# warwick-hpsc/MG-CFD-app-plain

Hardware: AMD Instinct MI355X
Metric: Medges/s (compute_flux_edge) + MG V-cycle wall-s (higher is better)
Workload: dtype f64; 1 GPU; M6-L0-like synthetic level (67^3 jittered lattice, permuted ids): 300763 nodes / 888822 internal edges per GPU, flux + update sweep, no MG; numerics=exact (bit-identical to the reference), parallelism=1 GPU, workload_kind=level0

## Files before the change

include/mgcfd.h:

```cpp
#ifndef MGCFD_H
#define MGCFD_H

#include <stdint.h>

#ifdef __cplusplus
extern "C" {
#endif

#define MGCFD_NVAR 5
#define MGCFD_RK 3

#define MGCFD_MESH_FVCORR 0
#define MGCFD_MESH_M6_WING 2
#define MGCFD_MESH_LA_CASCADE 3
#define MGCFD_MESH_ROTOR_37 4

#define MGCFD_OK 0
#define MGCFD_ERR_ARG 1
#define MGCFD_ERR_IO 2
#define MGCFD_ERR_HIP 3
#define MGCFD_ERR_NAN 4
#define MGCFD_ERR_NEG_DENSITY 5
#define MGCFD_ERR_NEG_ENERGY 6
#define MGCFD_ERR_VALIDATION 7
// ... 1 lines not shown
enum { MGCFD_LOOP_FLUX = 0, MGCFD_LOOP_UPDATE, MGCFD_LOOP_COMPUTE_STEP, MGCFD_LOOP_TIME_STEP,
       MGCFD_LOOP_RESTRICT, MGCFD_LOOP_PROLONG, MGCFD_LOOP_INDIRECT_RW, MGCFD_NUM_LOOPS };

enum { MGCFD_ARR_VARIABLES = 0, MGCFD_ARR_OLD_VARIABLES, MGCFD_ARR_FLUXES, MGCFD_ARR_RESIDUALS,
       MGCFD_ARR_STEP_FACTORS, MGCFD_ARR_VOLUMES,
       MGCFD_ARR_STAGE  };

enum {
    MGCFD_OPT_EXACT = 0,
    MGCFD_OPT_TIMING = 1,
    MGCFD_OPT_INDIRECT_RW = 2,
    MGCFD_OPT_CHECK_INVALID = 3,
    MGCFD_OPT_FLUX_VARIANT = 4,
    MGCFD_OPT_FUSE_UPDATE = 5,
    MGCFD_OPT_GRAPH = 6,
    MGCFD_OPT_RANK_SPLIT = 7
};

typedef struct { int64_t a, b; double x, y, z; } mgcfd_edge;

typedef struct {
    int64_t nel;
    int64_t n_edges;
    int64_t n_internal, n_boundary, n_wall;
    int64_t internal_start, boundary_start, wall_start;
    const double *volumes;
    const double *coords;
    const mgcfd_edge *edges;
    const int64_t *mg_map;
    int64_t mgc;
} mgcfd_level_desc;
// ... 20 lines not shown

int mgcfd_create(const mgcfd_level_desc *levels, int nlevels, int mesh_variant, int device,
                 mgcfd_solver **out);
int mgcfd_create_from_mesh(const mgcfd_mesh *m, int device, mgcfd_solver **out);
int mgcfd_create_partitioned(const mgcfd_level_desc *levels, int nlevels, int mesh_variant, int device,
                             const int64_t *n_owned, mgcfd_solver **out);
int mgcfd_create_partitioned_mg(const mgcfd_level_desc *levels, int nlevels, int mesh_variant, int device,
                                const int64_t *n_owned, const int64_t *const *order_keys, mgcfd_solver **out);
int mgcfd_plan_audit(const mgcfd_level_desc *levels, int nlevels, int mesh_variant, const int64_t *n_owned,
                     const int64_t *const *order_keys, char *report, int64_t report_cap);
void mgcfd_destroy(mgcfd_solver *s);
int mgcfd_set_option(mgcfd_solver *s, int option, int value);
int mgcfd_level_has_edge_once(const mgcfd_solver *s, int level, int *yes);
int mgcfd_level_has_half_rows(const mgcfd_solver *s, int level, int *yes);
int mgcfd_level_has_order_free(const mgcfd_solver *s, int level, int *yes);
int mgcfd_level_tiling(const mgcfd_solver *s, int level, int64_t out[10]);
int mgcfd_get_option(const mgcfd_solver *s, int option, int *value);
int mgcfd_set_stream(mgcfd_solver *s, void *hip_stream);
int mgcfd_synchronize(mgcfd_solver *s);
int mgcfd_num_levels(const mgcfd_solver *s);
int64_t mgcfd_level_nel(const mgcfd_solver *s, int level);
int64_t mgcfd_level_num_internal_edges(const mgcfd_solver *s, int level);
int mgcfd_get_far_field(const mgcfd_solver *s, double *out17);

int mgcfd_copy_old_variables(mgcfd_solver *s, int level);
int mgcfd_compute_step_factor(mgcfd_solver *s, int level);
int mgcfd_compute_flux_edge(mgcfd_solver *s, int level);
int mgcfd_compute_boundary_flux_edge(mgcfd_solver *s, int level);
int mgcfd_compute_wall_flux_edge(mgcfd_solver *s, int level);
int mgcfd_compute_fluxes(mgcfd_solver *s, int level);
// ... 78 lines not shown
```

mg-cfd-app-plain_amd/csrc/device_plan.hpp:

```cpp
#pragma once

#include <hip/hip_runtime.h>
#include <cstdint>

#include "preprocess.hpp"

namespace mgcfd {

constexpr int kNumStateFields = 5;
static_assert(sizeof(EdgeW) == 32, "EdgeW must be 32 bytes");
static_assert(sizeof(ProlongW) == 24, "ProlongW must be 24 bytes");

struct FarField {
    double var[5];
    double fc_mx[3], fc_my[3], fc_mz[3], fc_de[3];
};

constexpr int kMaxPushPeers = 8;
struct PushPeers {
    double *base[kMaxPushPeers] = {nullptr, nullptr, nullptr, nullptr, nullptr, nullptr, nullptr, nullptr};
    int64_t stride[kMaxPushPeers] = {0, 0, 0, 0, 0, 0, 0, 0};
    int64_t first[kMaxPushPeers + 1] = {0, 0, 0, 0, 0, 0, 0, 0, 0};
    int n = 0;
};

struct PushFlags {
// ... 96 lines not shown
    int64_t n_edges = 0, n_edges_pad = 0;
    int32_t *fe_ab = nullptr, *row_edge = nullptr;
    double *fe_w = nullptr, *edge_flux = nullptr;
    int32_t *old_of_new = nullptr;
    int32_t *child_ptr = nullptr, *child = nullptr;
    int32_t *child4 = nullptr;
    double *pro_w = nullptr;
    int32_t *pro_p = nullptr;
    int pro_tiled = 0;
    int32_t *pro_tile_n = nullptr, *pro_tile_ids = nullptr;
    uint16_t *pro_s16 = nullptr, *pro_own16 = nullptr;
    int32_t *pro_parent = nullptr;
    double *pro_wsum = nullptr;
};

}
```

mg-cfd-app-plain_amd/csrc/kernels.hip:

```cpp
#include <hip/hip_runtime.h>
#include <algorithm>
#include <cstdlib>
#include <stdexcept>
#include <stdint.h>

#include "device_plan.hpp"

#ifndef MGCFD_KERNEL_NS
#error "compile with -DMGCFD_KERNEL_NS=exact|fast"
#endif

namespace mgcfd {
namespace MGCFD_KERNEL_NS {

#ifdef MGCFD_PHASES
__device__ unsigned long long g_phase[4096 * 8];
__device__ unsigned long long g_phase_abs[4096 * 8];
#define PH_MARK(k) do { if (threadIdx.x == 0) { unsigned long long now_ = wall_clock64(); g_phase[(blockIdx.x & 4095) * 8 + (k)] += now_ - ph_last_; ph_last_ = now_; g_phase_abs[(blockIdx.x & 4095) * 8 + 1 + (k)] = now_; } } while (0)
#define PH_BEGIN() unsigned long long ph_last_ = wall_clock64(); if (threadIdx.x == 0) { g_phase[(blockIdx.x & 4095) * 8 + 7] += 1ull; g_phase_abs[(blockIdx.x & 4095) * 8] = ph_last_; \
        g_phase_abs[(blockIdx.x & 4095) * 8 + 7] = (static_cast<unsigned long long>(__builtin_amdgcn_s_getreg(20 | (0 << 6) | (31 << 11))) << 32) | __builtin_amdgcn_s_getreg(4 | (0 << 6) | (31 << 11)); }
#else
#define PH_MARK(k) do { } while (0)
#define PH_BEGIN() do { } while (0)
#endif
// ... 79 lines not shown
}

__device__ __forceinline__ NodeQ lds_load_record(const double2 *tile, uint32_t slot)
{
    const uint32_t b = (slot >> 3) & 1u;
    const double2 *even = tile + slot * kLdsRecD2 + b;
    const double2 *odd = tile + slot * kLdsRecD2 - b;
    const double2 a = even[0], bq = odd[1], c = even[2], d = odd[3], e = even[4];
    const double f = odd[5].x;
    NodeQ r;
    r.rho = a.x; r.mx = a.y; r.my = bq.x; r.mz = bq.y; r.en = c.x; r.vx = c.y;
    r.vy = d.x; r.vz = d.y; r.p = e.x; r.speed = e.y; r.c = f;
    return r;
}

struct FluxC { double xx, xy, xz, yy, yz, zz, ex, ey, ez; };

__device__ __forceinline__ FluxC flux_contribution(const NodeQ &q)
{
    FluxC f;
    f.xx = q.vx * q.mx + q.p;
    f.xy = q.vx * q.my;
    f.xz = q.vx * q.mz;
    f.yy = q.vy * q.my + q.p;
    f.yz = q.vy * q.mz;
    f.zz = q.vz * q.mz + q.p;
    const double de_p = q.en + q.p;
    f.ex = q.vx * de_p;
    f.ey = q.vy * de_p;
    f.ez = q.vz * de_p;
// ... 321 lines not shown
        } else if (e.code == kT16Far && (classes & 4)) {
            a0 += fx * (ff.var[1] + me.mx) + fy * (ff.var[2] + me.my) + fz * (ff.var[3] + me.mz);
            a4 += fx * (ff.fc_de[0] + fm.ex) + fy * (ff.fc_de[1] + fm.ey) + fz * (ff.fc_de[2] + fm.ez);
            a1 += fx * (ff.fc_mx[0] + fm.xx) + fy * (ff.fc_mx[1] + fm.xy) + fz * (ff.fc_mx[2] + fm.xz);
            a2 += fx * (ff.fc_my[0] + fm.xy) + fy * (ff.fc_my[1] + fm.yy) + fz * (ff.fc_my[2] + fm.yz);
            a3 += fx * (ff.fc_mz[0] + fm.xz) + fy * (ff.fc_mz[1] + fm.yz) + fz * (ff.fc_mz[2] + fm.zz);
        }
    }
}

struct FluxTileLds {
    double2 tile[kTileCap * kLdsRecD2];
    double s_pm[kBlock / 64];
    double s_next[2][kBlock / 64];
};

template <int WMODE, bool FUSE, bool ACC, int ROLE, bool TAIL, bool PUSH>
__device__ __forceinline__ void
flux_tile_body(FluxTileLds &lds, const unsigned block,
               const double *__restrict__ q, const int32_t *__restrict__ tile_halo, uint32_t n_tiles, int32_t pad_row,
               int64_t stride, int64_t nel, const int32_t *__restrict__ slice_row0,
               const int32_t *__restrict__ rows_int, const int32_t *__restrict__ rows_bnd,
               const uint16_t *__restrict__ nbr16, const double *__restrict__ w,
               const int32_t *__restrict__ tile_ovf_ptr, const int32_t *__restrict__ tile_ovf, const FarField &ff,
               double *__restrict__ fluxes, int classes, const FusedStep &fs, const TailPlan &tp,
               const uint16_t *__restrict__ gat16, const int32_t *__restrict__ te_chunk_ptr, const double *__restrict__ te_w3,
               const StagePush &push ,
               const bool block_is_tile = false )
{
    constexpr bool LOADK = WMODE == 1;
    static_assert(!PUSH || FUSE, "only a fused stage sends its message");
    PH_BEGIN();
    constexpr bool IDXW = WMODE == 2;
    static_assert(!(IDXW && TAIL), "indexed weights: levels without long rows only");
    double2 *const tile = lds.tile;

    double min_dt = 0.0;
    constexpr int kPartPre = 6;
    double *const s_pm = lds.s_pm;
    double pmv[kPartPre];

    const int tid = threadIdx.x;
    const int lane = tid & 63;
    unsigned t = block_is_tile ? block : xcd_contiguous_block(block, n_tiles);
    if (PUSH) {
        const unsigned nb = unsigned(push.n_boundary);
        t = block < nb ? block : nb + xcd_contiguous_block(block - nb, n_tiles - nb);
    }
    if (FUSE && fs.tile_list) t = unsigned(fs.tile_list[t]);
    const int64_t base = int64_t(t) * kTile;
    const int64_t i = base + tid;
    const int32_t slice = __builtin_amdgcn_readfirstlane(static_cast<int32_t>(i >> 6));

    const int32_t *hrow = tile_halo + int64_t(t) * kHaloStride;
    const int32_t hid = hrow[tid];
    const int32_t hid2 = (ROLE != 5 && tid < kHaloStride - kBlock) ? hrow[kBlock + tid] : -1;
    const int32_t row0 = slice_row0[slice];
    const int32_t n_int = (classes & 1) ? (TAIL ? tp.rows_main : rows_int)[slice] : 0;
    const int32_t n_bnd = rows_bnd[slice];
    const bool has_halo = hid >= 0;
    const int64_t hnode = has_halo ? int64_t(hid) : i;
    double o0, o1, o2, o3, o4, g0, g1, g2, g3, g4;
    EdgeRow e0, e1;
    RowRef i0{}, i1{}, i2{}, i3{};
    const double *tw = nullptr;
    if (IDXW) {
        i0 = load_ref(nbr16, gat16, n_int > 0 ? row0 : pad_row, lane);
        i1 = load_ref(nbr16, gat16, n_int > 1 ? row0 + 1 : pad_row, lane);
        i2 = load_ref(nbr16, gat16, n_int > 2 ? row0 + 2 : pad_row, lane);
        i3 = load_ref(nbr16, gat16, n_int > 3 ? row0 + 3 : pad_row, lane);
        tw = te_w3 + int64_t(te_chunk_ptr[t]) * (kEdgeChunk * 3);
// ... 32 lines not shown
        g0 = c0 + fh * h0; g1 = c1 + fh * h1; g2 = c2 + fh * h2; g3 = c3 + fh * h3; g4 = c4 + fh * h4;
        if (fs.check_vin && i < nel) {
            const bool finite = isfinite(o0) && isfinite(o1) && isfinite(o2) && isfinite(o3) && isfinite(o4);
            int code = 0;
            if (!finite) code = 1;
            else if (o0 < 0.0) code = 2;
            else if (o4 < 0.0) code = 3;
            if (code) atomicMin(fs.err, err_key(fs.check_vin, fs.old_of_new[i], code));
        }
    } else {
        o0 = q[i]; o1 = q[stride + i]; o2 = q[2 * stride + i]; o3 = q[3 * stride + i]; o4 = q[4 * stride + i];
        g0 = q[hnode]; g1 = q[stride + hnode]; g2 = q[2 * stride + hnode]; g3 = q[3 * stride + hnode]; g4 = q[4 * stride + hnode];
        if (IDXW) { e0 = gather_weights(tw, i0); e1 = gather_weights(tw, i1); }
        else {
            e0 = load_row<LOADK>(nbr16, w, n_int > 0 ? row0 : pad_row, lane);
            e1 = load_row<LOADK>(nbr16, w, n_int > 1 ? row0 + 1 : pad_row, lane);
        }
    }
    if (FUSE && ROLE == 0) {
#pragma unroll
        for (int u = 0; u < kPartPre; u++) {
            const int k = threadIdx.x + u * kBlock;
            pmv[u] = fs.partial_min[k < fs.n_partial ? k : fs.n_partial - 1];
        }
    }
    const NodeQ me = make_nodeq(o0, o1, o2, o3, o4);
    lds_store_record(tile, uint32_t(tid), me);
    lds_store_record(tile, uint32_t(kTile + tid), make_nodeq(g0, g1, g2, g3, g4));
    if (hid2 >= 0) lds_store_record(tile, uint32_t(kTile + kBlock + tid), load_and_derive(q, stride, hid2));

    const FluxC fm_pre = flux_contribution(me);
    double a0 = 0.0, a1 = 0.0, a2 = 0.0, a3 = 0.0, a4 = 0.0;
    if (ACC) {
        a0 = fluxes[i]; a1 = fluxes[stride + i]; a2 = fluxes[2 * stride + i];
        a3 = fluxes[3 * stride + i]; a4 = fluxes[4 * stride + i];
    }
    const int32_t ovf0 = tile_ovf_ptr[t];
    if (FUSE && ROLE == 0) {
        double pm = pmv[0];
#pragma unroll
        for (int u = 1; u < kPartPre; u++) pm = fmin(pm, pmv[u]);
        for (int k = threadIdx.x + kPartPre * kBlock; k < fs.n_partial; k += kBlock) pm = fmin(pm, fs.partial_min[k]);
        pm = wave_min(pm);
// ... 28 lines not shown
                a3 = v1 ? a3 + f1.mz : a3;  a4 = v1 ? a4 + f1.en : a4;                                       \
            } else {                                                                                         \
                a0 += f0.d; a1 += f0.mx; a2 += f0.my; a3 += f0.mz; a4 += f0.en;                              \
                a0 += f1.d; a1 += f1.mx; a2 += f1.my; a3 += f1.mz; a4 += f1.en;                              \
            }                                                                                                \
    } while (0)
    int32_t tl_b = 0, tl_e = 0, tl_nb = 0, tl_nc = 0;
    double2 tl_r0 = make_double2(0.0, 0.0), tl_r1 = tl_r0, tl_r2 = tl_r0;
    if (TAIL && (classes & 1)) {
        tl_b = tp.tile_ptr[t]; tl_e = tp.tile_ptr[t + 1];
        tl_nb = tp.begin[i]; tl_nc = tp.count[i];
        const int32_t e_first = tl_b + tid;
        if (e_first < tl_e) { tl_r0 = tp.rec[3 * int64_t(e_first)]; tl_r1 = tp.rec[3 * int64_t(e_first) + 1]; tl_r2 = tp.rec[3 * int64_t(e_first) + 2]; }
    }
    double r0 = 0.0, r1 = 0.0, r2 = 0.0, r3 = 0.0, r4 = 0.0, sfv = 0.0;
    {
        int32_t r = 0;
        if (IDXW) {
            for (; r + 2 < n_int; r += 2) {
                const RowRef i4 = load_ref(nbr16, gat16, r + 4 < n_int ? row0 + r + 4 : pad_row, lane);
                const RowRef i5 = load_ref(nbr16, gat16, r + 5 < n_int ? row0 + r + 5 : pad_row, lane);
                const EdgeRow e2 = gather_weights(tw, i2), e3 = gather_weights(tw, i3);
                MGCFD_ROW_PAIR();
                e0 = e2; e1 = e3; i2 = i4; i3 = i5;
            }
        } else
        for (; r + 2 < n_int; r += 2) {
            const EdgeRow e2 = load_row<LOADK>(nbr16, w, row0 + r + 2, lane);
            const EdgeRow e3 = load_row<LOADK>(nbr16, w, r + 3 < n_int ? row0 + r + 3 : pad_row, lane);
            MGCFD_ROW_PAIR();
            e0 = e2; e1 = e3;
        }
        if (FUSE) {
            if (ROLE == 0) {
                r0 = me.rho; r1 = me.mx; r2 = me.my; r3 = me.mz; r4 = me.en;
            } else {
                r0 = fs.old_variables[i]; r1 = fs.old_variables[stride + i]; r2 = fs.old_variables[2 * stride + i];
                r3 = fs.old_variables[3 * stride + i]; r4 = fs.old_variables[4 * stride + i];
            }
            sfv = ((ROLE == 0 || ROLE == 5) ? fs.volumes : fs.step_factors)[i];
        }
        if (r < n_int) MGCFD_ROW_PAIR();
    }
#undef MGCFD_ROW_PAIR
    PH_MARK(2);

    if (TAIL && (classes & 1) && tl_e > tl_b) {
        const int32_t last0 = tl_b + ((tl_e - tl_b - 1) / kBlock) * kBlock;
        int32_t e = tl_b + tid;
        double2 r0 = tl_r0, r1 = tl_r1, r2 = tl_r2;
        Flux5 fl;
        fl.d = 0.0; fl.mx = 0.0; fl.my = 0.0; fl.mz = 0.0; fl.en = 0.0;
        while (e < tl_e) {
            const double2 c0 = r0, c1 = r1, c2 = r2;
            const int32_t en = e + kBlock;
            if (en < tl_e) { r0 = tp.rec[3 * int64_t(en)]; r1 = tp.rec[3 * int64_t(en) + 1]; r2 = tp.rec[3 * int64_t(en) + 2]; }
            const uint32_t word = static_cast<uint32_t>(__double_as_longlong(c2.x));
            const uint32_t own = word & 0xFFFFu;
            if (own != kT16Pad) {
// ... 147 lines not shown
        double (*const s_next)[kBlock / 64] = lds.s_next;
        if (ROLE == 3) sf_next = wave_min(sf_next);
        if (fs.sumsq_partial) ss = wave_sum(ss);
        if ((threadIdx.x & 63) == 0) { s_next[0][threadIdx.x >> 6] = sf_next; s_next[1][threadIdx.x >> 6] = ss; }
        __syncthreads();
        if (threadIdx.x == 0) {
            double m = s_next[0][0], sum = s_next[1][0];
            for (int wv = 1; wv < kBlock / 64; wv++) { m = fmin(m, s_next[0][wv]); sum += s_next[1][wv]; }
            if (ROLE == 3) fs.next_partial_min[t] = m;
            if (fs.sumsq_partial) fs.sumsq_partial[t] = sum;
        }
    }
    PH_MARK(3);
}

template <int MINW, int WMODE, bool FUSE, bool ACC, int ROLE, bool TAIL, bool PUSH = false>
__global__ void __launch_bounds__(kBlock, MINW)
k_flux_tile(
            const double *__restrict__ q, const int32_t *__restrict__ tile_halo, uint32_t n_tiles, int32_t pad_row,
            int64_t stride, int64_t nel, const int32_t *__restrict__ slice_row0,
            const int32_t *__restrict__ rows_int, const int32_t *__restrict__ rows_bnd,
            const uint16_t *__restrict__ nbr16, const double *__restrict__ w,
            const int32_t *__restrict__ tile_ovf_ptr, const int32_t *__restrict__ tile_ovf, FarField ff,
            double *__restrict__ fluxes, int classes, FusedStep fs, TailPlan tp,
            const uint16_t *__restrict__ gat16, const int32_t *__restrict__ te_chunk_ptr, const double *__restrict__ te_w3,
            StagePush push)
{
    __shared__ FluxTileLds lds;
    flux_tile_body<WMODE, FUSE, ACC, ROLE, TAIL, PUSH>(lds, blockIdx.x, q, tile_halo, n_tiles, pad_row, stride, nel, slice_row0, rows_int, rows_bnd, nbr16, w,
                                                       tile_ovf_ptr, tile_ovf, ff, fluxes, classes, fs, tp, gat16, te_chunk_ptr, te_w3, push);
}

struct TileEdge { uint32_t sa, sb; double fx, fy, fz, k; };
constexpr int kGatherPre = 8;

template <bool LOADK>
__device__ __forceinline__ TileEdge load_tile_edge(const uint16_t *__restrict__ te_slots, const double *__restrict__ te_w,
                                                   int64_t chunk, int tid)
{
    TileEdge e;
    e.sa = te_slots[(chunk * 2) * kEdgeChunk + tid];
    e.sb = te_slots[(chunk * 2 + 1) * kEdgeChunk + tid];
    const double *wr = te_w + chunk * (4 * kEdgeChunk) + tid;
    e.fx = wr[0]; e.fy = wr[kEdgeChunk]; e.fz = wr[2 * kEdgeChunk];
// ... 1398 lines not shown
#define MGCFD_EO_LAUNCH(LOADK, FUSE, ACC)                                                                      \
    hipLaunchKernelGGL((k_flux_edge_once<LOADK, FUSE, ACC>), grid, block, 0, st, q, p.tile_halo,               \
                       uint32_t(p.n_tiles), p.pad_row, p.stride, p.nel, p.te_chunk_ptr, p.te_count,            \
                       p.pad_chunk, classes, p.slice_row0, p.rows_int, p.rows_bnd, p.nbr16, p.w, p.gat16,      \
                       p.te_slots, p.te_w, p.tile_ovf_ptr, p.tile_ovf, ff, fluxes, fs)
        if (fused) {
            if (loadk) MGCFD_EO_LAUNCH(true, true, false); else MGCFD_EO_LAUNCH(false, true, false);
        } else if (accumulate) {
            if (loadk) MGCFD_EO_LAUNCH(true, false, true); else MGCFD_EO_LAUNCH(false, false, true);
        } else {
            if (loadk) MGCFD_EO_LAUNCH(true, false, false); else MGCFD_EO_LAUNCH(false, false, false);
        }
#undef MGCFD_EO_LAUNCH
        return;
    }
    if (fused) {
        if (loadk) MGCFD_TILE_LAUNCH(true, true, false); else MGCFD_TILE_LAUNCH(false, true, false);
    } else if (accumulate) {
        if (loadk) MGCFD_TILE_LAUNCH(true, false, true); else MGCFD_TILE_LAUNCH(false, false, true);
    } else {
        if (loadk) MGCFD_TILE_LAUNCH(true, false, false); else MGCFD_TILE_LAUNCH(false, false, false);
    }
#undef MGCFD_TILE_LAUNCH
#undef MGCFD_TILE_LAUNCH_R
#undef MGCFD_TILE_LAUNCH_T
}

__global__ void __launch_bounds__(kBlock)
k_stream_tiles(const double2 *__restrict__ src, double *__restrict__ dst, int64_t rd_total2, int64_t wr_total, int rd2_per_thread, int wr_per_thread)
{
// ... 140 lines not shown
```

mg-cfd-app-plain_amd/csrc/preprocess.hpp:

```cpp
#pragma once

#include <cstdint>
#include <string>
#include <vector>

#include "mgcfd.h"

namespace mgcfd {

constexpr int kSlice = 64;
constexpr int kTile = 256;
constexpr int kTileCap = 559;
constexpr int kHaloStride = kTileCap - kTile;
static_assert(kTileCap >= 2 * kTile, "every thread has a halo slot (the kernels stage one unconditionally)");
static_assert(kHaloStride <= 2 * kTile, "the staging code reads at most two halo ids per thread");
constexpr int kProCap = 768;
constexpr int kEdgeChunk = 256;
constexpr int kMaxEdgeChunks = 5;
constexpr uint32_t kHalfForeign = 1u << 24;
constexpr uint32_t kHalfMirror = 1u << 25;
constexpr uint32_t kHalfPad = 0x00007FFFu;
constexpr int kHalfMaxRows = 5;
constexpr int kFreeHaloStride = 2 * kTile;
constexpr int kFreeCap4Halo = 290;
constexpr int kFreeMaxRows = 32;
constexpr int kHalfTileRows = 21;
constexpr int kHalfSlots = kHalfTileRows * kSlice;
// ... 105 lines not shown
```

mg-cfd-app-plain_amd/csrc/solver.cpp:

```cpp
#include <hip/hip_runtime.h>
#include <dlfcn.h>

#include <functional>
#include <future>

#include <algorithm>
#include <atomic>
#include <cmath>
#include <cstdio>
#include <cstdlib>
#include <chrono>
#include <cstring>
#include <limits>
#include <map>
#include <memory>
#include <mutex>
#include <stdexcept>
#include <string>
#include <thread>
#include <vector>

#include "kernels.hpp"
#include "mesh.hpp"
#include "mgcfd.h"
// ... 144 lines not shown

}

using namespace mgcfd;

struct mgcfd_mesh { HostMesh mesh; };

struct mgcfd_solver {
    int device = 0;
    int mesh_variant = 0;
    hipStream_t own_stream = nullptr, stream = nullptr;
    std::vector<DeviceLevel> L;
    FarField ff{};
    double ff17[17] = {0};
    unsigned long long *err = nullptr;
    int opt_exact = 1, opt_timing = 0, opt_indirect_rw = 0, opt_check = 1, opt_variant = -1, opt_fuse = 1, opt_graph = 0;
    int opt_rank_split = 1;
    bool opt_lazy_residual = !(std::getenv("MGCFD_LAZY_RESIDUAL") && std::atoi(std::getenv("MGCFD_LAZY_RESIDUAL")) == 0);
    int check_seq = 0;
    int64_t invalid_cell = -1; int invalid_cycle = -1;
    int next_check() { if (!opt_check) return 0; if (check_seq < (1 << 22)) check_seq++; return check_seq; }
    int force_check = -1;
    int timing_stride = 8;
    double att_total = 0.0;
    bool probe_first_stage_only = false;
    int64_t sweep_counter = 0;
    bool in_timed_group = false;
    struct SweepGraph { hipGraphExec_t exec = nullptr; int64_t iters[MGCFD_NUM_LOOPS] = {0}; bool ahead_after = false; int rot_after = 0; int sf_par_after = 0; bool sumsq_after = false, res_stale_after = false; };
    std::map<uint64_t, SweepGraph> sweep_graphs;
    struct CycleGraph { hipGraphExec_t exec = nullptr; std::vector<std::vector<int64_t>> iters; std::vector<bool> ahead_after, res_stale_after; std::vector<int> rot_after, sf_par_after; };
    std::map<uint64_t, CycleGraph> cycle_graphs;
// ... 140 lines not shown
        }
        if (!lv.dp.nbr && ((v >= 0 && (v & 8)) || !lv.dp.lds_complete || lv.dp.has_tail)) lv.dp.nbr = take(P.nbr);
    }
    void upload_optional_plans()
    {
        use_device();
        for (DeviceLevel &lv : L) upload_optional_plans(lv);
    }
    int variant_for(const DeviceLevel &lv, bool fused = false) const
    {
        if (opt_variant >= 0) return opt_variant;
        const bool free_fast_path = !lv.dp.free_wide && lv.dp.halo_max <= kFreeCap4Halo && lv.dp.hr_max_rows <= kHalfMaxRows;
        if (!opt_exact && lv.dp.free_rows && (!fused || lv.dp.free_wide || lv.dp.has_tail || free_fast_path)) return 1 | 64;
        return 1;
    }
    void op_flux(int l, int classes)
    {
        DeviceLevel &lv = level(l);
        Timed t(this, l, MGCFD_LOOP_FLUX, (classes & 1) != 0);
        if (classes != 7) settle_fluxes(lv);
        const int accumulate = lv.fluxes_zero ? 0 : 1;
        const int variant = variant_for(lv);
        if ((variant & 4) && !lv.dp.edge_flux)
            lv.dp.edge_flux = dev_alloc<double>(static_cast<size_t>(lv.dp.n_edges_pad) * 5 + 8);
        if (opt_exact) exact::launch_flux(stream, lv.dp, lv.q, ff, lv.fluxes, classes, accumulate, variant, nullptr);
        else fast::launch_flux(stream, lv.dp, lv.q, ff, lv.fluxes, classes, accumulate, variant, nullptr);
        lv.fluxes_zero = false;
        lv.fluxes_stale = false;
        if (classes & 1) lv.iters[MGCFD_LOOP_FLUX] += lv.info.n_internal;
    }
    void op_fused_stage(int l, int j, const double *in, double *out, int apply_min, bool with_residual,
                        const double *old = nullptr, bool look_ahead = false, bool sumsq = false,
                        const double *vin_flux = nullptr, const int32_t *tile_list = nullptr, int32_t n_list = 0,
                        bool count_iters = true, const double *min_list = nullptr, int n_min = 0, bool lazy_residual = false,
                        const StagePush *push = nullptr)
    {
        DeviceLevel &lv = level(l);
        const FusedStep fs = fused_step(l, j, out, apply_min, with_residual, old, look_ahead, sumsq, vin_flux, tile_list, n_list, min_list, n_min, lazy_residual);
        Timed t(this, l, MGCFD_LOOP_FLUX, true);
        if (opt_exact) exact::launch_flux(stream, lv.dp, in, ff, lv.fluxes, 7, 0, variant_for(lv, true), &fs, push);
        else fast::launch_flux(stream, lv.dp, in, ff, lv.fluxes, 7, 0, variant_for(lv, true), &fs, push);
        if (count_iters) {
            lv.iters[MGCFD_LOOP_FLUX] += lv.info.n_internal;
            lv.iters[MGCFD_LOOP_TIME_STEP] += lv.info.nel;
        }
    }
    FusedStep fused_step(int l, int j, double *out, int apply_min, bool with_residual, const double *old, bool look_ahead, bool sumsq,
                         const double *vin_flux, const int32_t *tile_list, int32_t n_list, const double *min_list, int n_min, bool lazy_residual)
    {
        DeviceLevel &lv = level(l);
        settle_residuals(lv);
        FusedStep fs;
        fs.tile_list = tile_list;
        fs.n_list = n_list;
        if (tile_list && lv.plan.ghosts_last && lv.n_owned < lv.info.nel) fs.nel_active = lv.n_owned;
// ... 636 lines not shown
    REQUIRE(s);
    return guarded([&] {
        switch (option) {
            case MGCFD_OPT_EXACT: s->opt_exact = value != 0; s->upload_optional_plans(); break;
            case MGCFD_OPT_TIMING:
                if (value < 0 || value > 4) throw std::invalid_argument("MGCFD_OPT_TIMING is 0 ... 4");
                s->use_device(); s->fold_events(); s->opt_timing = value == 3 ? 2 : value; s->timing_stride = value == 3 ? 1 : (value == 4 ? 32 : 8);
                if (const char *e = std::getenv("MGCFD_TIMING_STRIDE")) if (std::atoi(e) > 0 && value != 3) s->timing_stride = std::atoi(e);
                break;
            case MGCFD_OPT_INDIRECT_RW: s->opt_indirect_rw = value != 0; break;
            case MGCFD_OPT_CHECK_INVALID: s->opt_check = value != 0; break;
            case MGCFD_OPT_FLUX_VARIANT: s->opt_variant = value; s->upload_optional_plans(); break;
            case MGCFD_OPT_FUSE_UPDATE: s->opt_fuse = value != 0; break;
            case MGCFD_OPT_GRAPH: s->opt_graph = value != 0; break;
            case MGCFD_OPT_RANK_SPLIT: s->opt_rank_split = value < 0 ? 0 : (value > 2 ? 2 : value); break;
            default: throw std::invalid_argument("unknown option");
        }
    });
}
int mgcfd_level_has_half_rows(const mgcfd_solver *s, int level, int *yes)
{
    REQUIRE(s); REQUIRE(yes);
    if (level < 0 || level >= static_cast<int>(s->L.size())) { g_last_error = "level out of range"; return MGCFD_ERR_ARG; }
    *yes = s->L[static_cast<size_t>(level)].dp.half;
    return MGCFD_OK;
}
int mgcfd_level_has_order_free(const mgcfd_solver *s, int level, int *yes)
{
    REQUIRE(s); REQUIRE(yes);
    if (level < 0 || level >= static_cast<int>(s->L.size())) { g_last_error = "level out of range"; return MGCFD_ERR_ARG; }
    *yes = s->L[static_cast<size_t>(level)].dp.free_rows;
    return MGCFD_OK;
}
int mgcfd_level_has_edge_once(const mgcfd_solver *s, int level, int *yes)
{
    REQUIRE(s); REQUIRE(yes);
    if (level < 0 || level >= static_cast<int>(s->L.size())) { g_last_error = "level out of range"; return MGCFD_ERR_ARG; }
    *yes = s->L[static_cast<size_t>(level)].dp.edge_once;
    return MGCFD_OK;
}
int mgcfd_level_tiling(const mgcfd_solver *s, int level, int64_t out[10])
{
    REQUIRE(s); REQUIRE(out);
    if (level < 0 || level >= static_cast<int>(s->L.size())) { g_last_error = "level out of range"; return MGCFD_ERR_ARG; }
    const LevelPlan &P = s->L[static_cast<size_t>(level)].plan;
    out[0] = P.n_tiles;
// ... 9 lines not shown
    for (int32_t r : P.rows_main) out[9] += r;
    return MGCFD_OK;
}
int mgcfd_get_option(const mgcfd_solver *s, int option, int *value)
{
    REQUIRE(s); REQUIRE(value);
    switch (option) {
        case MGCFD_OPT_EXACT: *value = s->opt_exact; break;
        case MGCFD_OPT_TIMING: *value = s->opt_timing; break;
        case MGCFD_OPT_INDIRECT_RW: *value = s->opt_indirect_rw; break;
        case MGCFD_OPT_CHECK_INVALID: *value = s->opt_check; break;
        case MGCFD_OPT_FLUX_VARIANT: *value = s->opt_variant; break;
        case MGCFD_OPT_FUSE_UPDATE: *value = s->opt_fuse; break;
        case MGCFD_OPT_GRAPH: *value = s->opt_graph; break;
        case MGCFD_OPT_RANK_SPLIT: *value = s->opt_rank_split; break;
        default: g_last_error = "unknown option"; return MGCFD_ERR_ARG;
    }
    return MGCFD_OK;
}
int mgcfd_set_stream(mgcfd_solver *s, void *hip_stream)
{
    REQUIRE(s);
    return guarded([&] {
        s->use_device();
        s->fold_events();
        HIP_CHECK(hipStreamSynchronize(s->stream));
        s->stream = hip_stream ? static_cast<hipStream_t>(hip_stream) : s->own_stream;
    });
}
int mgcfd_synchronize(mgcfd_solver *s)
// ... 147 lines not shown
        if (keep_p) lv.iters[MGCFD_LOOP_INDIRECT_RW] += int64_t(probe ? MGCFD_RK - 1 : MGCFD_RK) * lv.info.n_internal;
        if (!probe) s->opt_indirect_rw = 0;
        s->probe_first_stage_only = true;
        try { smooth_once(s, level); } catch (...) { s->opt_timing = keep_t; s->opt_indirect_rw = keep_p; s->probe_first_stage_only = false; throw; }
        s->opt_timing = keep_t; s->opt_indirect_rw = keep_p; s->probe_first_stage_only = false;
        return;
    }
    const bool graphable = s->opt_graph && s->opt_fuse && !(s->variant_for(lv) & 4) && !s->opt_indirect_rw && !timed && lv.fluxes_zero && !lv.fluxes_stale;
    if (!graphable) {
        const int keep = s->opt_timing;
        if (!timed) s->opt_timing = 0;
        smooth_once(s, level);
        s->opt_timing = keep;
        return;
    }
    const uint64_t key = (uint64_t(level) << 32) | (uint64_t(lv.want_sumsq) << 28) | (uint64_t(lv.sf_par) << 27) | (uint64_t(lv.rot) << 25) | (uint64_t(lv.min_ahead) << 24) | (uint64_t(s->opt_exact) << 16) | (uint64_t(s->opt_check) << 8) | uint64_t(s->opt_variant & 0xFF);
    auto it = s->sweep_graphs.find(key);
    if (it == s->sweep_graphs.end()) {
        mgcfd_solver::SweepGraph g;
        int64_t before[MGCFD_NUM_LOOPS];
        std::memcpy(before, lv.iters, sizeof(before));
        const int keep = s->opt_timing;
        s->opt_timing = 0;
        hipGraph_t graph = nullptr;
        HIP_CHECK(hipStreamBeginCapture(s->stream, hipStreamCaptureModeRelaxed));
        try {
            smooth_once(s, level);
        } catch (...) {
            (void)hipStreamEndCapture(s->stream, &graph);
            if (graph) (void)hipGraphDestroy(graph);
            s->opt_timing = keep;
// ... 184 lines not shown
        }
        const size_t nl = s->L.size();
        std::vector<double> sums;
        sums.reserve(static_cast<size_t>(cycles > 0 ? cycles : 0));
        seq_before = s->check_seq;
        for (int done = 0; done < cycles;) {
            const int chunk = std::min(cycles - done, mgcfd_solver::kRmsRing);
            HIP_CHECK(hipMemsetAsync(s->rms_count, 0, sizeof(int), s->stream));
            hipEvent_t att0 = nullptr, att1 = nullptr;
            if (s->opt_timing == 4) { att0 = s->get_event(); att1 = s->get_event(); HIP_CHECK(hipEventRecord(att0, s->stream)); }
            bool graphable = s->opt_graph && s->opt_fuse && !s->opt_indirect_rw && s->opt_timing == 0;
            for (auto &lv : s->L) graphable = graphable && lv.fluxes_zero && !lv.fluxes_stale && !(s->variant_for(lv) & 4);
            graphable = graphable && nl <= 8;
            if (graphable) {
                for (int c = 0; c < chunk; c++) {
                    uint64_t key = (uint64_t(s->opt_exact) << 16) | (uint64_t(s->opt_check) << 8) | uint64_t(s->opt_variant & 0xFF);
                    for (size_t l = 0; l < nl && l < 8; l++) key |= (uint64_t(s->L[l].min_ahead) << (24 + l)) | (uint64_t(s->L[l].rot) << (32 + 2 * l)) | (uint64_t(s->L[l].sf_par) << (48 + l));
                    auto it = s->cycle_graphs.find(key);
                    if (it == s->cycle_graphs.end()) {
                        mgcfd_solver::CycleGraph g;
                        std::vector<std::vector<int64_t>> before(nl);
                        std::vector<bool> ahead_before, stale_before;
                        std::vector<int> rot_before, sf_before;
                        for (size_t l = 0; l < nl; l++) {
                            before[l].assign(s->L[l].iters, s->L[l].iters + MGCFD_NUM_LOOPS);
                            ahead_before.push_back(s->L[l].min_ahead);
                            stale_before.push_back(s->L[l].residuals_stale);
                            rot_before.push_back(s->L[l].rot);
                            sf_before.push_back(s->L[l].sf_par);
                        }
                        hipGraph_t graph = nullptr;
// ... 1848 lines not shown
```

mg-cfd-app-plain_amd/mgcfd/api.py:

```python
from __future__ import annotations

import ctypes as C
import os
import sys
from typing import List, Optional, Sequence

import numpy as np

from .meshgen import EDGE_DTYPE, LevelMesh, MultigridMesh, to_edge_arrays

PKG_DIR = os.path.dirname(os.path.abspath(__file__))
CSRC_DIR = os.path.normpath(os.path.join(PKG_DIR, "..", "csrc"))
LIB_PATH = os.environ.get("MGCFD_LIB") or os.path.join(CSRC_DIR, "libmgcfd_hip.so")

NVAR = 5
RK = 3
LOOPS = ("flux", "update", "compute_step", "time_step", "restrict", "prolong", "indirect_rw")
ARR = {"variables": 0, "old_variables": 1, "fluxes": 2, "residuals": 3, "step_factors": 4, "volumes": 5, "stage": 6}
OPT = {"exact": 0, "timing": 1, "indirect_rw": 2, "check_invalid": 3, "flux_variant": 4, "fuse_update": 5, "graph": 6, "rank_split": 7}
ERR_NAMES = {0: "OK", 1: "ERR_ARG", 2: "ERR_IO", 3: "ERR_HIP", 4: "ERR_NAN", 5: "ERR_NEG_DENSITY",
             6: "ERR_NEG_ENERGY", 7: "ERR_VALIDATION"}

_vp = C.c_void_p
_i64 = C.c_int64


class LevelDesc(C.Structure):
    _fields_ = [("nel", _i64), ("n_edges", _i64), ("n_internal", _i64), ("n_boundary", _i64),
                ("n_wall", _i64), ("internal_start", _i64), ("boundary_start", _i64), ("wall_start", _i64),
                ("volumes", _vp), ("coords", _vp), ("edges", _vp), ("mg_map", _vp), ("mgc", _i64)]


class MgcfdError(RuntimeError):
    def __init__(self, code: int, message: str):
# ... 16 lines not shown
    ("mgcfd_create", C.c_int, [C.POINTER(LevelDesc), C.c_int, C.c_int, C.c_int, C.POINTER(_vp)]),
    ("mgcfd_plan_audit", C.c_int, [C.POINTER(LevelDesc), C.c_int, C.c_int, C.POINTER(_i64), C.POINTER(C.POINTER(_i64)), C.c_char_p, _i64]),
    ("mgcfd_create_partitioned_mg", C.c_int, [C.POINTER(LevelDesc), C.c_int, C.c_int, C.c_int, C.POINTER(_i64),
                                                 C.POINTER(C.POINTER(_i64)), C.POINTER(_vp)]),
    ("mgcfd_create_from_mesh", C.c_int, [_vp, C.c_int, C.POINTER(_vp)]),
    ("mgcfd_create_partitioned", C.c_int, [C.POINTER(LevelDesc), C.c_int, C.c_int, C.c_int, C.POINTER(_i64), C.POINTER(_vp)]),
    ("mgcfd_halo_plan", C.c_int, [_vp, C.c_int, _i64, _vp, C.POINTER(C.c_int)]),
    ("mgcfd_halo_pack", C.c_int, [_vp, C.c_int, C.c_int, C.c_int, _vp]),
    ("mgcfd_halo_unpack", C.c_int, [_vp, C.c_int, C.c_int, C.c_int, _vp]),
    ("mgcfd_destroy", None, [_vp]),
    ("mgcfd_set_option", C.c_int, [_vp, C.c_int, C.c_int]),
    ("mgcfd_level_has_edge_once", C.c_int, [_vp, C.c_int, C.POINTER(C.c_int)]),
    ("mgcfd_level_has_half_rows", C.c_int, [_vp, C.c_int, C.POINTER(C.c_int)]),
    ("mgcfd_pending_invalid_state", C.c_int, [_vp, C.POINTER(C.c_int64)]),
    ("mgcfd_level_has_order_free", C.c_int, [_vp, C.c_int, C.POINTER(C.c_int)]),
    ("mgcfd_level_tiling", C.c_int, [_vp, C.c_int, C.POINTER(C.c_int64)]),
    ("mgcfd_invalid_state_location", C.c_int, [_vp, C.POINTER(C.c_int64), C.POINTER(C.c_int)]),
    ("mgcfd_get_option", C.c_int, [_vp, C.c_int, C.POINTER(C.c_int)]),
    ("mgcfd_set_stream", C.c_int, [_vp, _vp]),
    ("mgcfd_synchronize", C.c_int, [_vp]),
    ("mgcfd_num_levels", C.c_int, [_vp]),
    ("mgcfd_level_nel", _i64, [_vp, C.c_int]),
    ("mgcfd_level_num_internal_edges", _i64, [_vp, C.c_int]),
    ("mgcfd_get_far_field", C.c_int, [_vp, _vp]),
    ("mgcfd_copy_old_variables", C.c_int, [_vp, C.c_int]),
    ("mgcfd_compute_step_factor", C.c_int, [_vp, C.c_int]),
    ("mgcfd_compute_flux_edge", C.c_int, [_vp, C.c_int]),
    ("mgcfd_compute_boundary_flux_edge", C.c_int, [_vp, C.c_int]),
    ("mgcfd_compute_wall_flux_edge", C.c_int, [_vp, C.c_int]),
    ("mgcfd_compute_fluxes", C.c_int, [_vp, C.c_int]),
# ... 259 lines not shown
        self._c(self.lib.mgcfd_level_tiling(self.handle, l, out))
        keys = ("tiles", "halo_nodes", "halo_max", "halo_capacity", "overflow_refs", "row_entries", "padding_entries", "coordinate_boxes",
                "list_entries", "loop_rows")
        return dict(zip(keys, (int(v) for v in out)))

    def has_half_rows(self, l: int) -> bool:
        yes = C.c_int(0)
        self._c(self.lib.mgcfd_level_has_half_rows(self.handle, l, C.byref(yes)))
        return bool(yes.value)

    def has_order_free(self, l: int) -> bool:
        yes = C.c_int(0)
        self._c(self.lib.mgcfd_level_has_order_free(self.handle, l, C.byref(yes)))
        return bool(yes.value)

    def has_edge_once(self, l: int) -> bool:
        v = C.c_int()
        self._c(self.lib.mgcfd_level_has_edge_once(self.handle, l, C.byref(v)))
        return bool(v.value)

    def get_option(self, name: str) -> int:
        v = C.c_int()
        self._c(self.lib.mgcfd_get_option(self.handle, OPT[name], C.byref(v)))
        return v.value

    def set_stream(self, stream_handle: Optional[int]):
        if stream_handle is not None and int(stream_handle) == 0:
            raise ValueError("stream handle 0 is the legacy default stream; make a torch.cuda.Stream() current "
                             "(torch.cuda.set_stream) and pass its .cuda_stream, or pass None for the solver's own stream")
        self._c(self.lib.mgcfd_set_stream(self.handle, _vp(stream_handle) if stream_handle is not None else None))
# ... 261 lines not shown
```

Baseline: 51220 Medges/s.

## Add slim 80-byte LDS records so fused flux stages fit four workgroups per CU

Adds a SLIM variant of the fused tile flux kernel. It stores node records in LDS as 80 bytes instead of the larger format and recomputes pressure on load. The tile capacity is capped at 510 so the LDS struct fits four workgroups per CU, with launch bounds set to 4. The inner loop processes one row at a time with a prefetch instead of row pairs, trading ILP for occupancy. The path is enabled by default in exact mode when the level has no tail, its halo fits, and it has more than three tiles per CU.

```diff
diff --git a/include/mgcfd.h b/include/mgcfd.h
--- a/include/mgcfd.h
+++ b/include/mgcfd.h
@@ -39,7 +39,8 @@
     MGCFD_OPT_FLUX_VARIANT = 4,
     MGCFD_OPT_FUSE_UPDATE = 5,
     MGCFD_OPT_GRAPH = 6,
-    MGCFD_OPT_RANK_SPLIT = 7
+    MGCFD_OPT_RANK_SPLIT = 7,
+    MGCFD_OPT_STAGE_WG4 = 8
 };
 
 typedef struct { int64_t a, b; double x, y, z; } mgcfd_edge;
@@ -90,6 +91,7 @@
 int mgcfd_level_has_edge_once(const mgcfd_solver *s, int level, int *yes);
 int mgcfd_level_has_half_rows(const mgcfd_solver *s, int level, int *yes);
 int mgcfd_level_has_order_free(const mgcfd_solver *s, int level, int *yes);
+int mgcfd_level_stage_wg4(const mgcfd_solver *s, int level, int *yes);
 int mgcfd_level_tiling(const mgcfd_solver *s, int level, int64_t out[10]);
 int mgcfd_get_option(const mgcfd_solver *s, int option, int *value);
 int mgcfd_set_stream(mgcfd_solver *s, void *hip_stream);
diff --git a/mg-cfd-app-plain_amd/csrc/device_plan.hpp b/mg-cfd-app-plain_amd/csrc/device_plan.hpp
--- a/mg-cfd-app-plain_amd/csrc/device_plan.hpp
+++ b/mg-cfd-app-plain_amd/csrc/device_plan.hpp
@@ -10,6 +10,8 @@
 constexpr int kNumStateFields = 5;
 static_assert(sizeof(EdgeW) == 32, "EdgeW must be 32 bytes");
 static_assert(sizeof(ProlongW) == 24, "ProlongW must be 24 bytes");
+
+constexpr int kVariantStageWg4 = 1 << 7;
 
 struct FarField {
     double var[5];
@@ -136,4 +138,6 @@
     double *pro_wsum = nullptr;
 };
 
+inline bool stage_wg4_fits(const DevicePlan &p) { return !p.has_tail && p.halo_max <= kTileCap4 - kTile; }
+
 }
diff --git a/mg-cfd-app-plain_amd/csrc/kernels.hip b/mg-cfd-app-plain_amd/csrc/kernels.hip
--- a/mg-cfd-app-plain_amd/csrc/kernels.hip
+++ b/mg-cfd-app-plain_amd/csrc/kernels.hip
@@ -3,6 +3,7 @@
 #include <cstdlib>
 #include <stdexcept>
 #include <stdint.h>
+#include <type_traits>
 
 #include "device_plan.hpp"
 
@@ -117,6 +118,42 @@
     return r;
 }
 
+constexpr int kLdsRec80D2 = 5;
+
+__device__ __forceinline__ void lds_put_record80(double2 *tile, uint32_t slot, const NodeQ &n)
+{
+    double2 *rec = tile + slot * kLdsRec80D2;
+    rec[0] = make_double2(n.rho, n.mx);
+    rec[1] = make_double2(n.my, n.mz);
+    rec[2] = make_double2(n.en, n.vx);
+    rec[3] = make_double2(n.vy, n.vz);
+    rec[4] = make_double2(n.speed, n.c);
+}
+
+__device__ __forceinline__ NodeQ lds_get_record80(const double2 *tile, uint32_t slot)
+{
+    const double2 *rec = tile + slot * kLdsRec80D2;
+    const double2 a = rec[0], b = rec[1], c = rec[2], d = rec[3], e = rec[4];
+    NodeQ r;
+    r.rho = a.x; r.mx = a.y; r.my = b.x; r.mz = b.y; r.en = c.x; r.vx = c.y;
+    r.vy = d.x; r.vz = d.y; r.speed = e.x; r.c = e.y;
+    r.p = (kGamma - 1.0) * (r.en - 0.5 * r.rho * (r.vx * r.vx + r.vy * r.vy + r.vz * r.vz));
+    return r;
+}
+
+template <bool SLIM>
+__device__ __forceinline__ void lds_put_rec(double2 *tile, uint32_t slot, const NodeQ &n)
+{
+    if (SLIM) lds_put_record80(tile, slot, n);
+    else lds_store_record(tile, slot, n);
+}
+
+template <bool SLIM>
+__device__ __forceinline__ NodeQ lds_get_rec(const double2 *tile, uint32_t slot)
+{
+    return SLIM ? lds_get_record80(tile, slot) : lds_load_record(tile, slot);
+}
+
 struct FluxC { double xx, xy, xz, yy, yz, zz, ex, ey, ez; };
 
 __device__ __forceinline__ FluxC flux_contribution(const NodeQ &q)
@@ -468,10 +505,17 @@
     double s_pm[kBlock / 64];
     double s_next[2][kBlock / 64];
 };
-
-template <int WMODE, bool FUSE, bool ACC, int ROLE, bool TAIL, bool PUSH>
+struct FluxTileLds4 {
+    double2 tile[kTileCap4 * kLdsRec80D2];
+    double s_pm[kBlock / 64];
+    double s_next[2][kBlock / 64];
+};
+static_assert(sizeof(FluxTileLds4) <= 160 * 1024 / 4, "four workgroups per CU");
+static_assert(kTileCap4 - kTile < kBlock, "one halo id per thread");
+
+template <int WMODE, bool FUSE, bool ACC, int ROLE, bool TAIL, bool PUSH, bool SLIM = false, typename Lds = FluxTileLds>
 __device__ __forceinline__ void
-flux_tile_body(FluxTileLds &lds, const unsigned block,
+flux_tile_body(Lds &lds, const unsigned block,
                const double *__restrict__ q, const int32_t *__restrict__ tile_halo, uint32_t n_tiles, int32_t pad_row,
                int64_t stride, int64_t nel, const int32_t *__restrict__ slice_row0,
                const int32_t *__restrict__ rows_int, const int32_t *__restrict__ rows_bnd,
@@ -487,6 +531,7 @@
     PH_BEGIN();
     constexpr bool IDXW = WMODE == 2;
     static_assert(!(IDXW && TAIL), "indexed weights: levels without long rows only");
+    static_assert(!SLIM || (!TAIL && !IDXW && !PUSH && ROLE != 5), "80-byte records: the stages without long rows, indexed weights, message or absorbed stage");
     double2 *const tile = lds.tile;
 
     double min_dt = 0.0;
@@ -508,7 +553,7 @@
 
     const int32_t *hrow = tile_halo + int64_t(t) * kHaloStride;
     const int32_t hid = hrow[tid];
-    const int32_t hid2 = (ROLE != 5 && tid < kHaloStride - kBlock) ? hrow[kBlock + tid] : -1;
+    const int32_t hid2 = (!SLIM && ROLE != 5 && tid < kHaloStride - kBlock) ? hrow[kBlock + tid] : -1;
     const int32_t row0 = slice_row0[slice];
     const int32_t n_int = (classes & 1) ? (TAIL ? tp.rows_main : rows_int)[slice] : 0;
     const int32_t n_bnd = rows_bnd[slice];
@@ -571,7 +616,7 @@
         if (IDXW) { e0 = gather_weights(tw, i0); e1 = gather_weights(tw, i1); }
         else {
             e0 = load_row<LOADK>(nbr16, w, n_int > 0 ? row0 : pad_row, lane);
-            e1 = load_row<LOADK>(nbr16, w, n_int > 1 ? row0 + 1 : pad_row, lane);
+            if (!SLIM) e1 = load_row<LOADK>(nbr16, w, n_int > 1 ? row0 + 1 : pad_row, lane);
         }
     }
     if (FUSE && ROLE == 0) {
@@ -582,8 +627,9 @@
         }
     }
     const NodeQ me = make_nodeq(o0, o1, o2, o3, o4);
-    lds_store_record(tile, uint32_t(tid), me);
-    lds_store_record(tile, uint32_t(kTile + tid), make_nodeq(g0, g1, g2, g3, g4));
+    lds_put_rec<SLIM>(tile, uint32_t(tid), me);
+    const uint32_t hslot = (SLIM && tid >= kTileCap4 - kTile) ? uint32_t(tid) : uint32_t(kTile + tid);
+    lds_put_rec<SLIM>(tile, hslot, make_nodeq(g0, g1, g2, g3, g4));
     if (hid2 >= 0) lds_store_record(tile, uint32_t(kTile + kBlock + tid), load_and_derive(q, stride, hid2));
 
     const FluxC fm_pre = flux_contribution(me);
@@ -642,6 +688,37 @@
         if (e_first < tl_e) { tl_r0 = tp.rec[3 * int64_t(e_first)]; tl_r1 = tp.rec[3 * int64_t(e_first) + 1]; tl_r2 = tp.rec[3 * int64_t(e_first) + 2]; }
     }
     double r0 = 0.0, r1 = 0.0, r2 = 0.0, r3 = 0.0, r4 = 0.0, sfv = 0.0;
+#define MGCFD_ROW_ONE()                                                                                      \
+    do {                                                                                                     \
+            const uint32_t s0 = e0.code & kT16SlotMask;                                                      \
+            const bool v0 = s0 != kT16Pad;                                                                   \
+            const NodeQ n0 = lds_get_record80(tile, v0 ? s0 : uint32_t(tid));                              \
+            const Flux5 f0 = edge_flux<LOADK>(me, fm_pre, n0, e0);                                           \
+            if (ACC) {                                                                                       \
+                a0 = v0 ? a0 + f0.d : a0;   a1 = v0 ? a1 + f0.mx : a1;   a2 = v0 ? a2 + f0.my : a2;          \
+                a3 = v0 ? a3 + f0.mz : a3;  a4 = v0 ? a4 + f0.en : a4;                                       \
+            } else {                                                                                         \
+                a0 += f0.d; a1 += f0.mx; a2 += f0.my; a3 += f0.mz; a4 += f0.en;                              \
+            }                                                                                                \
+    } while (0)
+    if (SLIM) {
+        int32_t r = 0;
+        for (; r + 1 < n_int; r++) {
+            const EdgeRow e1n = load_row<LOADK>(nbr16, w, row0 + r + 1, lane);
+            MGCFD_ROW_ONE();
+            e0 = e1n;
+        }
+        if (FUSE) {
+            if (ROLE == 0) {
+                r0 = me.rho; r1 = me.mx; r2 = me.my; r3 = me.mz; r4 = me.en;
+            } else {
+                r0 = fs.old_variables[i]; r1 = fs.old_variables[stride + i]; r2 = fs.old_variables[2 * stride + i];
+                r3 = fs.old_variables[3 * stride + i]; r4 = fs.old_variables[4 * stride + i];
+            }
+            sfv = (ROLE == 0 ? fs.volumes : fs.step_factors)[i];
+        }
+        if (r < n_int) MGCFD_ROW_ONE();
+    } else
     {
         int32_t r = 0;
         if (IDXW) {
@@ -671,6 +748,7 @@
         if (r < n_int) MGCFD_ROW_PAIR();
     }
 #undef MGCFD_ROW_PAIR
+#undef MGCFD_ROW_ONE
     PH_MARK(2);
 
     if (TAIL && (classes & 1) && tl_e > tl_b) {
@@ -848,7 +926,7 @@
     PH_MARK(3);
 }
 
-template <int MINW, int WMODE, bool FUSE, bool ACC, int ROLE, bool TAIL, bool PUSH = false>
+template <int MINW, int WMODE, bool FUSE, bool ACC, int ROLE, bool TAIL, bool PUSH = false, bool SLIM = false>
 __global__ void __launch_bounds__(kBlock, MINW)
 k_flux_tile(
             const double *__restrict__ q, const int32_t *__restrict__ tile_halo, uint32_t n_tiles, int32_t pad_row,
@@ -860,8 +938,8 @@
             const uint16_t *__restrict__ gat16, const int32_t *__restrict__ te_chunk_ptr, const double *__restrict__ te_w3,
             StagePush push)
 {
-    __shared__ FluxTileLds lds;
-    flux_tile_body<WMODE, FUSE, ACC, ROLE, TAIL, PUSH>(lds, blockIdx.x, q, tile_halo, n_tiles, pad_row, stride, nel, slice_row0, rows_int, rows_bnd, nbr16, w,
+    __shared__ std::conditional_t<SLIM, FluxTileLds4, FluxTileLds> lds;
+    flux_tile_body<WMODE, FUSE, ACC, ROLE, TAIL, PUSH, SLIM>(lds, blockIdx.x, q, tile_halo, n_tiles, pad_row, stride, nel, slice_row0, rows_int, rows_bnd, nbr16, w,
                                                        tile_ovf_ptr, tile_ovf, ff, fluxes, classes, fs, tp, gat16, te_chunk_ptr, te_w3, push);
 }
 
@@ -2290,6 +2368,27 @@
 #undef MGCFD_EO_LAUNCH
         return;
     }
+#ifndef MGCFD_ORDER_FREE
+    if (fused && (variant & kVariantStageWg4) && stage_wg4_fits(p) && !indexed && role != 5) {
+#define MGCFD_SLIM_LAUNCH_T(WMODE, ROLE)                                                                        \
+    hipLaunchKernelGGL((k_flux_tile<4, WMODE, true, false, ROLE, false, false, true>), grid, block, 0, st, q, p.tile_halo, \
+                       uint32_t(grid.x), p.pad_row, p.stride, nel_arg, p.slice_row0, p.rows_int, p.rows_bnd, \
+                       p.nbr16, p.w, p.tile_ovf_ptr, p.tile_ovf, ff, fluxes, classes, fs, p.tail, p.gat16,     \
+                       p.te_chunk_ptr, p.te_w3, StagePush{})
+#define MGCFD_SLIM_LAUNCH_R(WMODE)                                                                              \
+    do {                                                                                                       \
+        if (role == 0) MGCFD_SLIM_LAUNCH_T(WMODE, 0);                                                          \
+        else if (role == 2) MGCFD_SLIM_LAUNCH_T(WMODE, 2);                                                     \
+        else if (role == 3) MGCFD_SLIM_LAUNCH_T(WMODE, 3);                                                     \
+        else if (role == 4) MGCFD_SLIM_LAUNCH_T(WMODE, 4);                                                     \
+        else MGCFD_SLIM_LAUNCH_T(WMODE, 1);                                                                    \
+    } while (0)
+        if (loadk) MGCFD_SLIM_LAUNCH_R(1); else MGCFD_SLIM_LAUNCH_R(0);
+#undef MGCFD_SLIM_LAUNCH_R
+#undef MGCFD_SLIM_LAUNCH_T
+        return;
+    }
+#endif
     if (fused) {
         if (loadk) MGCFD_TILE_LAUNCH(true, true, false); else MGCFD_TILE_LAUNCH(false, true, false);
     } else if (accumulate) {
diff --git a/mg-cfd-app-plain_amd/csrc/preprocess.hpp b/mg-cfd-app-plain_amd/csrc/preprocess.hpp
--- a/mg-cfd-app-plain_amd/csrc/preprocess.hpp
+++ b/mg-cfd-app-plain_amd/csrc/preprocess.hpp
@@ -11,6 +11,7 @@
 constexpr int kSlice = 64;
 constexpr int kTile = 256;
 constexpr int kTileCap = 559;
+constexpr int kTileCap4 = 510;
 constexpr int kHaloStride = kTileCap - kTile;
 static_assert(kTileCap >= 2 * kTile, "every thread has a halo slot (the kernels stage one unconditionally)");
 static_assert(kHaloStride <= 2 * kTile, "the staging code reads at most two halo ids per thread");
diff --git a/mg-cfd-app-plain_amd/csrc/solver.cpp b/mg-cfd-app-plain_amd/csrc/solver.cpp
--- a/mg-cfd-app-plain_amd/csrc/solver.cpp
+++ b/mg-cfd-app-plain_amd/csrc/solver.cpp
@@ -182,7 +182,7 @@
     FarField ff{};
     double ff17[17] = {0};
     unsigned long long *err = nullptr;
-    int opt_exact = 1, opt_timing = 0, opt_indirect_rw = 0, opt_check = 1, opt_variant = -1, opt_fuse = 1, opt_graph = 0;
+    int opt_exact = 1, opt_timing = 0, opt_indirect_rw = 0, opt_check = 1, opt_variant = -1, opt_fuse = 1, opt_graph = 0, opt_stage_wg4 = 1;
     int opt_rank_split = 1;
     bool opt_lazy_residual = !(std::getenv("MGCFD_LAZY_RESIDUAL") && std::atoi(std::getenv("MGCFD_LAZY_RESIDUAL")) == 0);
     int check_seq = 0;
@@ -353,6 +353,16 @@
         if (!opt_exact && lv.dp.free_rows && (!fused || lv.dp.free_wide || lv.dp.has_tail || free_fast_path)) return 1 | 64;
         return 1;
     }
+    mutable int n_cus = 0;
+    bool stage_wg4_for(const DeviceLevel &lv) const
+    {
+        if (!opt_exact || !opt_stage_wg4 || !stage_wg4_fits(lv.dp)) return false;
+        if (n_cus == 0) {
+            use_device();
+            HIP_CHECK(hipDeviceGetAttribute(&n_cus, hipDeviceAttributeMultiprocessorCount, device));
+        }
+        return lv.dp.n_tiles > 3 * n_cus;
+    }
     void op_flux(int l, int classes)
     {
         DeviceLevel &lv = level(l);
@@ -377,7 +387,7 @@
         DeviceLevel &lv = level(l);
         const FusedStep fs = fused_step(l, j, out, apply_min, with_residual, old, look_ahead, sumsq, vin_flux, tile_list, n_list, min_list, n_min, lazy_residual);
         Timed t(this, l, MGCFD_LOOP_FLUX, true);
-        if (opt_exact) exact::launch_flux(stream, lv.dp, in, ff, lv.fluxes, 7, 0, variant_for(lv, true), &fs, push);
+        if (opt_exact) exact::launch_flux(stream, lv.dp, in, ff, lv.fluxes, 7, 0, variant_for(lv, true) | (stage_wg4_for(lv) ? kVariantStageWg4 : 0), &fs, push);
         else fast::launch_flux(stream, lv.dp, in, ff, lv.fluxes, 7, 0, variant_for(lv, true), &fs, push);
         if (count_iters) {
             lv.iters[MGCFD_LOOP_FLUX] += lv.info.n_internal;
@@ -1044,6 +1054,7 @@
             case MGCFD_OPT_FUSE_UPDATE: s->opt_fuse = value != 0; break;
             case MGCFD_OPT_GRAPH: s->opt_graph = value != 0; break;
             case MGCFD_OPT_RANK_SPLIT: s->opt_rank_split = value < 0 ? 0 : (value > 2 ? 2 : value); break;
+            case MGCFD_OPT_STAGE_WG4: s->opt_stage_wg4 = value != 0; break;
             default: throw std::invalid_argument("unknown option");
         }
     });
@@ -1060,6 +1071,13 @@
     REQUIRE(s); REQUIRE(yes);
     if (level < 0 || level >= static_cast<int>(s->L.size())) { g_last_error = "level out of range"; return MGCFD_ERR_ARG; }
     *yes = s->L[static_cast<size_t>(level)].dp.free_rows;
+    return MGCFD_OK;
+}
+int mgcfd_level_stage_wg4(const mgcfd_solver *s, int level, int *yes)
+{
+    REQUIRE(s); REQUIRE(yes);
+    if (level < 0 || level >= static_cast<int>(s->L.size())) { g_last_error = "level out of range"; return MGCFD_ERR_ARG; }
+    *yes = s->stage_wg4_for(s->L[static_cast<size_t>(level)]) ? 1 : 0;
     return MGCFD_OK;
 }
 int mgcfd_level_has_edge_once(const mgcfd_solver *s, int level, int *yes)
@@ -1099,6 +1117,7 @@
         case MGCFD_OPT_FUSE_UPDATE: *value = s->opt_fuse; break;
         case MGCFD_OPT_GRAPH: *value = s->opt_graph; break;
         case MGCFD_OPT_RANK_SPLIT: *value = s->opt_rank_split; break;
+        case MGCFD_OPT_STAGE_WG4: *value = s->opt_stage_wg4; break;
         default: g_last_error = "unknown option"; return MGCFD_ERR_ARG;
     }
     return MGCFD_OK;
@@ -1276,7 +1295,7 @@
         s->opt_timing = keep;
         return;
     }
-    const uint64_t key = (uint64_t(level) << 32) | (uint64_t(lv.want_sumsq) << 28) | (uint64_t(lv.sf_par) << 27) | (uint64_t(lv.rot) << 25) | (uint64_t(lv.min_ahead) << 24) | (uint64_t(s->opt_exact) << 16) | (uint64_t(s->opt_check) << 8) | uint64_t(s->opt_variant & 0xFF);
+    const uint64_t key = (uint64_t(level) << 32) | (uint64_t(lv.want_sumsq) << 28) | (uint64_t(lv.sf_par) << 27) | (uint64_t(lv.rot) << 25) | (uint64_t(lv.min_ahead) << 24) | (uint64_t(s->opt_exact) << 16) | (uint64_t(s->opt_stage_wg4) << 17) | (uint64_t(s->opt_check) << 8) | uint64_t(s->opt_variant & 0xFF);
     auto it = s->sweep_graphs.find(key);
     if (it == s->sweep_graphs.end()) {
         mgcfd_solver::SweepGraph g;
@@ -1491,7 +1510,7 @@
             graphable = graphable && nl <= 8;
             if (graphable) {
                 for (int c = 0; c < chunk; c++) {
-                    uint64_t key = (uint64_t(s->opt_exact) << 16) | (uint64_t(s->opt_check) << 8) | uint64_t(s->opt_variant & 0xFF);
+                    uint64_t key = (uint64_t(s->opt_exact) << 16) | (uint64_t(s->opt_stage_wg4) << 17) | (uint64_t(s->opt_check) << 8) | uint64_t(s->opt_variant & 0xFF);
                     for (size_t l = 0; l < nl && l < 8; l++) key |= (uint64_t(s->L[l].min_ahead) << (24 + l)) | (uint64_t(s->L[l].rot) << (32 + 2 * l)) | (uint64_t(s->L[l].sf_par) << (48 + l));
                     auto it = s->cycle_graphs.find(key);
                     if (it == s->cycle_graphs.end()) {
diff --git a/mg-cfd-app-plain_amd/mgcfd/api.py b/mg-cfd-app-plain_amd/mgcfd/api.py
--- a/mg-cfd-app-plain_amd/mgcfd/api.py
+++ b/mg-cfd-app-plain_amd/mgcfd/api.py
@@ -17,7 +17,7 @@
 RK = 3
 LOOPS = ("flux", "update", "compute_step", "time_step", "restrict", "prolong", "indirect_rw")
 ARR = {"variables": 0, "old_variables": 1, "fluxes": 2, "residuals": 3, "step_factors": 4, "volumes": 5, "stage": 6}
-OPT = {"exact": 0, "timing": 1, "indirect_rw": 2, "check_invalid": 3, "flux_variant": 4, "fuse_update": 5, "graph": 6, "rank_split": 7}
+OPT = {"exact": 0, "timing": 1, "indirect_rw": 2, "check_invalid": 3, "flux_variant": 4, "fuse_update": 5, "graph": 6, "rank_split": 7, "stage_wg4": 8}
 ERR_NAMES = {0: "OK", 1: "ERR_ARG", 2: "ERR_IO", 3: "ERR_HIP", 4: "ERR_NAN", 5: "ERR_NEG_DENSITY",
              6: "ERR_NEG_ENERGY", 7: "ERR_VALIDATION"}
 
@@ -64,6 +64,7 @@
     ("mgcfd_level_has_half_rows", C.c_int, [_vp, C.c_int, C.POINTER(C.c_int)]),
     ("mgcfd_pending_invalid_state", C.c_int, [_vp, C.POINTER(C.c_int64)]),
     ("mgcfd_level_has_order_free", C.c_int, [_vp, C.c_int, C.POINTER(C.c_int)]),
+    ("mgcfd_level_stage_wg4", C.c_int, [_vp, C.c_int, C.POINTER(C.c_int)]),
     ("mgcfd_level_tiling", C.c_int, [_vp, C.c_int, C.POINTER(C.c_int64)]),
     ("mgcfd_invalid_state_location", C.c_int, [_vp, C.POINTER(C.c_int64), C.POINTER(C.c_int)]),
     ("mgcfd_get_option", C.c_int, [_vp, C.c_int, C.POINTER(C.c_int)]),
@@ -353,6 +354,11 @@
         self._c(self.lib.mgcfd_level_has_order_free(self.handle, l, C.byref(yes)))
         return bool(yes.value)
 
+    def stage_wg4(self, l: int) -> bool:
+        yes = C.c_int(0)
+        self._c(self.lib.mgcfd_level_stage_wg4(self.handle, l, C.byref(yes)))
+        return bool(yes.value)
+
     def has_edge_once(self, l: int) -> bool:
         v = C.c_int()
         self._c(self.lib.mgcfd_level_has_edge_once(self.handle, l, C.byref(v)))
```

New measurement: 53910 Medges/s, median of 6. +5.3%, better.
